# zhoupengwei/tloam

Measured on AMD Instinct MI355X. Metric: gauss_newton_iters_per_sec, higher is better.
Workload: dtype f64

## Files before the change

tloam_amd/csrc/tl_walk.hpp:

```cpp
#pragma once

#include "tl_common.hpp"
#include "tl_knn.hpp"

#ifndef TL_K1_STAMP
#define TL_K1_STAMP(i)
#endif

namespace tl {

template <int K, int LPQ>
__device__ __forceinline__ void knn_rows(const GridView& g, const PtsGlobal& pts, Vec3 pw, int sub, TopK<K>& tk,
                                         int2* __restrict__ lds_rows, double radius, NbrXyz<K>* xyz = nullptr) {
  TL_K1_STAMP(1)
  const int cx = cell_coord(pw.x, g.org[0], g.inv_cell, g.dim[0]);
  const int cy = cell_coord(pw.y, g.org[1], g.inv_cell, g.dim[1]);
  const int cz = cell_coord(pw.z, g.org[2], g.inv_cell, g.dim[2]);
  int x0 = cx - 1;
  if (x0 < 0) x0 = 0;
  constexpr int NR = (9 + LPQ - 1) / LPQ;
  int rs[NR], re[NR];
  const double cl = g.cell, reach = radius * (1.0 + 1e-6), c2 = reach * reach;
  const double fx = (pw.x - g.org[0]) * g.inv_cell - (double)cx, fy = (pw.y - g.org[1]) * g.inv_cell - (double)cy,
               fz = (pw.z - g.org[2]) * g.inv_cell - (double)cz;
  const double dxl = fx * cl, dxr = (1.0 - fx) * cl, dyl = fy * cl, dyr = (1.0 - fy) * cl, dzl = fz * cl, dzr = (1.0 - fz) * cl;
  const double sxl = dxl * dxl, sxr = dxr * dxr, syl = dyl * dyl, syr = dyr * dyr, szl = dzl * dzl, szr = dzr * dzr;
  typedef int int4u __attribute__((ext_vector_type(4), aligned(4)));
#pragma unroll
  for (int i = 0; i < NR; ++i) {
    const int r = sub + i * LPQ;
    const int rz = r / 3, ry = r % 3;
    const int z = cz - 1 + rz, y = cy - 1 + ry;
    const double s2 = (rz == 0 ? szl : (rz == 2 ? szr : 0.0)) + (ry == 0 ? syl : (ry == 2 ? syr : 0.0));
    int xa = cx - ((s2 + sxl <= c2) ? 1 : 0), xb = cx + ((s2 + sxr <= c2) ? 1 : 0);
    if (xa < 0) xa = 0;
    if (xb >= g.dim[0]) xb = g.dim[0] - 1;
    const bool in = (r < 9) && (s2 <= c2) && (xa <= xb) && z >= 0 && z < g.dim[2] && y >= 0 && y < g.dim[1];
    const size_t base = in ? ((size_t)z * g.dim[1] + y) * g.dim[0] + x0 : 0;
    const int4u t = *reinterpret_cast<const int4u*>(g.cell_start + base);
    const int ia = xa - x0, ib = xb + 1 - x0;
    rs[i] = in ? (ia == 0 ? t.x : t.y) : 0;
    re[i] = in ? (ib == 3 ? t.w : (ib == 2 ? t.z : t.y)) : 0;
  }
  topk_clear<K>(tk);
  TL_K1_STAMP(2)
  if (LPQ == 1) {
    const int lane = threadIdx.x & 63;
    int nr = 0, total = 0;
#pragma unroll
    for (int i = 0; i < NR; ++i) {
      const int len = re[i] - rs[i];
      if (len > 0) {
        lds_rows[nr * 64 + lane] = int2{rs[i], re[i]};
        ++nr;
        total += len;
      }
    }
    int j = 0, e = 0, r = 0;
    int2 nx = (nr > 0) ? lds_rows[lane] : int2{0, 0};
    const unsigned keep_mask = ~((1u << key_bits_for(g.n)) - 1u);
    KeyList<K + 1> L;
    keys_clear<K + 1>(L);
    auto next = [&](int& jx, bool& vx) {
      if (j >= e && r < nr) { j = nx.x; e = nx.y; ++r; nx = lds_rows[(r < nr ? r : 0) * 64 + lane]; }
      vx = j < e;
      jx = vx ? j : 0;
      j += vx ? 1 : 0;
    };
#ifndef TLOAM_K1_CPT
#define TLOAM_K1_CPT 4
#endif
    constexpr int kCpt = TLOAM_K1_CPT;
    int jc[kCpt];
    bool vc[kCpt];
    double4 rc[kCpt];
#pragma unroll
    for (int u = 0; u < kCpt; ++u) next(jc[u], vc[u]);
#pragma unroll
    for (int u = 0; u < kCpt; ++u) rc[u] = pts.p[jc[u]];
#ifdef TLOAM_K1_DBG_NOWALK
    total = 0;
#endif
#ifdef TLOAM_K1_DBG_MAXTRIPS
    int trip_no = 0;
    for (int left = total; __any(left > 0) && trip_no < TLOAM_K1_DBG_MAXTRIPS; left -= kCpt, ++trip_no) {
#else
    for (int left = total; __any(left > 0); left -= kCpt) {
#endif
      int jn[kCpt];
      bool vn[kCpt];
      double4 rn[kCpt];
#pragma unroll
      for (int u = 0; u < kCpt; ++u) next(jn[u], vn[u]);
#pragma unroll
      for (int u = 0; u < kCpt; ++u) rn[u] = pts.p[jn[u]];
#pragma unroll
      for (int u = 0; u < kCpt; ++u) {
        const double du = sqdist(pw.x, pw.y, pw.z, rc[u].x, rc[u].y, rc[u].z);
        key_insert<K + 1>(L, key_pack(du, jc[u], keep_mask, vc[u]));
      }
#pragma unroll
      for (int u = 0; u < kCpt; ++u) { jc[u] = jn[u]; vc[u] = vn[u]; rc[u] = rn[u]; }
    }
    if (!keys_ambiguous<K + 1>(L, keep_mask)) {
      keys_unpack<K, K + 1>(L, pts, pw.x, pw.y, pw.z, keep_mask, tk, xyz);
    } else {
      topk_clear<K>(tk);
      for (int q = 0; q < nr; ++q) {
        const int2 v = lds_rows[q * 64 + lane];
        scan_range<K>(pts, v.x, v.y, pw.x, pw.y, pw.z, tk);
      }
      if (xyz) nbr_fetch<K>(pts, tk, xyz);
    }
  } else {
    const unsigned keep_mask = ~((1u << key_bits_for(g.n)) - 1u);
    KeyList<K + 1> L;
    keys_clear<K + 1>(L);
    int len = 0;
#pragma unroll
    for (int i = 0; i < NR; ++i) len = max(len, re[i] - rs[i]);
#ifndef TLOAM_K1_WIDE_KU
#define TLOAM_K1_WIDE_KU 4
#endif
    constexpr int kU = (NR == 1) ? TLOAM_K1_WIDE_KU : 2;
#ifdef TLOAM_K1_DBG_NOWALK
    len = 0;
#endif
    for (int s = 0; s < len; s += kU) {
      double4 c[kU][NR];
#pragma unroll
      for (int u = 0; u < kU; ++u)
#pragma unroll
        for (int i = 0; i < NR; ++i) c[u][i] = pts.p[(rs[i] + s + u < re[i]) ? rs[i] + s + u : 0];
#pragma unroll
      for (int u = 0; u < kU; ++u)
#pragma unroll
        for (int i = 0; i < NR; ++i) {
          const bool v = rs[i] + s + u < re[i];
          key_insert<K + 1>(L, key_pack(sqdist(pw.x, pw.y, pw.z, c[u][i].x, c[u][i].y, c[u][i].z), rs[i] + s + u, keep_mask, v));
        }
    }
    TL_K1_STAMP(3)
#ifndef TLOAM_K1_DBG_NOMERGE
#pragma unroll
    for (int x = 1; x < LPQ; x <<= 1) {
      double ok[K + 1];
#pragma unroll
      for (int m = 0; m < K + 1; ++m) ok[m] = __shfl_xor(L.k[m], x, 64);
#pragma unroll
      for (int m = 0; m < K + 1; ++m) key_insert<K + 1>(L, ok[m]);
    }
#endif
    TL_K1_STAMP(4)
    if (!keys_ambiguous<K + 1>(L, keep_mask)) {
      keys_unpack<K, K + 1>(L, pts, pw.x, pw.y, pw.z, keep_mask, tk, xyz);
      TL_K1_STAMP(5)
    } else {
      for (int s = 0; s < len; ++s) {
        double4 c[NR];
#pragma unroll
        for (int i = 0; i < NR; ++i) c[i] = pts.p[(rs[i] + s < re[i]) ? rs[i] + s : 0];
#pragma unroll
        for (int i = 0; i < NR; ++i)
          if (rs[i] + s < re[i])
            topk_insert<K, PtsGlobal>(tk, pts, sqdist(pw.x, pw.y, pw.z, c[i].x, c[i].y, c[i].z), rs[i] + s);
      }
#pragma unroll
      for (int x = 1; x < LPQ; x <<= 1) {
        double od[K];
        int oj[K];
#pragma unroll
        for (int m = 0; m < K; ++m) { od[m] = __shfl_xor(tk.d[m], x, 64); oj[m] = __shfl_xor(tk.j[m], x, 64); }
#pragma unroll
        for (int m = 0; m < K; ++m)
          if (oj[m] >= 0) topk_insert<K, PtsGlobal>(tk, pts, od[m], oj[m]);
      }
      if (xyz) nbr_fetch<K>(pts, tk, xyz);
    }
  }
}

}
```

Baseline: 62130.

## Load-balance KNN row walk across lanes with DPP prefix scan and split loads

When each lane owns a single grid row (NR==1), the lanes of a 16-lane query group now compute a prefix sum of row lengths with DPP row shifts. They then cooperatively walk the concatenated candidate list, so each lane handles an equal share instead of the longest row setting the loop length. Each pair of lanes splits a 32-byte point load into two 16-byte halves and exchanges the z coordinate via a DPP swap, with only even lanes inserting keys. This trades per-candidate binary-search shuffles and extra DPP ops for better balance and less redundant memory traffic.

After: 64540 (median of 6 runs). 3.9% higher.

```diff
diff --git a/tloam_amd/csrc/tl_walk.hpp b/tloam_amd/csrc/tl_walk.hpp
--- a/tloam_amd/csrc/tl_walk.hpp
+++ b/tloam_amd/csrc/tl_walk.hpp
@@ -8,6 +8,11 @@
 #endif
 
 namespace tl {
+
+template <int CTRL>
+__device__ __forceinline__ int row_dpp(int v) {
+  return __builtin_amdgcn_update_dpp(0, v, CTRL, 0xf, 0xf, true);
+}
 
 template <int K, int LPQ>
 __device__ __forceinline__ void knn_rows(const GridView& g, const PtsGlobal& pts, Vec3 pw, int sub, TopK<K>& tk,
@@ -119,26 +124,62 @@
     int len = 0;
 #pragma unroll
     for (int i = 0; i < NR; ++i) len = max(len, re[i] - rs[i]);
-#ifndef TLOAM_K1_WIDE_KU
-#define TLOAM_K1_WIDE_KU 4
-#endif
-    constexpr int kU = (NR == 1) ? TLOAM_K1_WIDE_KU : 2;
+    if constexpr (NR == 1) {
+      const int ln = re[0] - rs[0];
+      int inc = ln;
+      inc += row_dpp<0x111>(inc);
+      inc += row_dpp<0x112>(inc);
+      inc += row_dpp<0x114>(inc);
+      inc += row_dpp<0x118>(inc);
+      const int pre_own = inc - ln, off_own = rs[0] - pre_own;
+      int T = row_dpp<0x15F>(inc);
 #ifdef TLOAM_K1_DBG_NOWALK
-    len = 0;
-#endif
-    for (int s = 0; s < len; s += kU) {
-      double4 c[kU][NR];
-#pragma unroll
-      for (int u = 0; u < kU; ++u)
-#pragma unroll
-        for (int i = 0; i < NR; ++i) c[u][i] = pts.p[(rs[i] + s + u < re[i]) ? rs[i] + s + u : 0];
-#pragma unroll
-      for (int u = 0; u < kU; ++u)
-#pragma unroll
-        for (int i = 0; i < NR; ++i) {
-          const bool v = rs[i] + s + u < re[i];
-          key_insert<K + 1>(L, key_pack(sqdist(pw.x, pw.y, pw.z, c[u][i].x, c[u][i].y, c[u][i].z), rs[i] + s + u, keep_mask, v));
+      T = 0;
+#endif
+      constexpr int kPc = 4;
+      const bool even = (sub & 1) == 0;
+      const char* const half0 = reinterpret_cast<const char*>(pts.p) + (sub & 1) * 16;
+      for (int b = 0; b < T; b += 8 * kPc) {
+        int jp[kPc];
+        bool vp[kPc];
+        double2 c[kPc];
+#pragma unroll
+        for (int u = 0; u < kPc; ++u) {
+          const int rec = b + u * 8 + (sub >> 1);
+          int row = 0;
+#pragma unroll
+          for (int st = 8; st >= 1; st >>= 1) row += (__shfl(pre_own, row + st, 16) <= rec) ? st : 0;
+          const int o = __shfl(off_own, row, 16);
+          vp[u] = rec < T;
+          jp[u] = vp[u] ? rec + o : 0;
         }
+#pragma unroll
+        for (int u = 0; u < kPc; ++u) c[u] = *reinterpret_cast<const double2*>(half0 + (size_t)jp[u] * sizeof(double4));
+#pragma unroll
+        for (int u = 0; u < kPc; ++u) {
+          const double z = __hiloint2double(row_dpp<0xB1>(__double2hiint(c[u].x)), row_dpp<0xB1>(__double2loint(c[u].x)));
+          key_insert<K + 1>(L, key_pack(sqdist(pw.x, pw.y, pw.z, c[u].x, c[u].y, z), jp[u], keep_mask, vp[u] && even));
+        }
+      }
+    } else {
+      constexpr int kU = 2;
+#ifdef TLOAM_K1_DBG_NOWALK
+      len = 0;
+#endif
+      for (int s = 0; s < len; s += kU) {
+        double4 c[kU][NR];
+#pragma unroll
+        for (int u = 0; u < kU; ++u)
+#pragma unroll
+          for (int i = 0; i < NR; ++i) c[u][i] = pts.p[(rs[i] + s + u < re[i]) ? rs[i] + s + u : 0];
+#pragma unroll
+        for (int u = 0; u < kU; ++u)
+#pragma unroll
+          for (int i = 0; i < NR; ++i) {
+            const bool v = rs[i] + s + u < re[i];
+            key_insert<K + 1>(L, key_pack(sqdist(pw.x, pw.y, pw.z, c[u][i].x, c[u][i].y, c[u][i].z), rs[i] + s + u, keep_mask, v));
+          }
+      }
     }
     TL_K1_STAMP(3)
 #ifndef TLOAM_K1_DBG_NOMERGE
```
